# kai0511/insider

Measured on AMD Instinct MI355X. Metric: outer-iterations/sec (masked INSIDER fit, 10000 x 50000, K=30), higher is better.
Workload: dtype f64

## Files before the change

### insider_amd/csrc/insider_hip.hip

```cpp
#include "insider_kernels.hpp"
#include "insider_posthoc.hpp"
#include "insider_vardecomp.hpp"
#include "insider_sampdecomp.hpp"
#include "insider_levelscores.hpp"
#include "insider_factdecomp.hpp"
#include "insider_rescomp.hpp"
#include "insider_outliers.hpp"
#include "insider_neighbors.hpp"
#include "insider_coexpr.hpp"
#include "insider_enrich.hpp"
#include "insider_kmeans.hpp"
#include "insider_tsne.hpp"

#include <rccl/rccl.h>

#include <algorithm>
#include <chrono>
#include <cstdlib>
#include <cmath>
#include <cstdio>
#include <cstring>
#include <limits>
#include <memory>
#include <mutex>
// ... 222 lines not shown
    int blocks() const { return c + (m > 0 ? 1 : 0); }
    Block block(int b) const { return b < c ? Block{n_levels[b], lvl_off[b]} : Block{m, SLcat}; }

    DataSet() = default;
    DataSet(const DataSet &) = delete;
    DataSet &operator=(const DataSet &) = delete;
    ~DataSet() { (void)hipSetDevice(device); }
};

struct Workspace {
    static constexpr int EARLY = 3;
    int K = 0, NB = 0, KP = 0, nseg = 1;
    int gram_blocks_p = 0, gram_blocks_n = 0, sc_blocks = 0;
    DevBuf<double> Astack, R, C, RtR, CCt, Qfull, SC, stat, stat_col, gram_part, sc_part, lvl_part, eq, lvl_sum;
    DevBuf<double> fperm;
    DevBuf<double> lvl_zero;
    DevBuf<double> Qheld;
    DevBuf<double> U, Ylvl, wpart, Vlev;
    DevBuf<double> lvl_sum_all;
    DevBuf<double> gram_part2, sc_part2;
    DevBuf<double> wg_part;
    DevBuf<uint8_t> wg_pair;
    DevBuf<double> sse_train, sse_test, b2, b1, loss_buf, stage;
    size_t stage_count = 0;
    DevBuf<int> sweeps, failflag;
    DevBuf<int> sweep_key;
    DevBuf<unsigned long long> sweep_total;
    DevBuf<unsigned> pc4_ticket;
    unsigned pc4_base[2] = {0, 0};
    unsigned long long cd_code_base = 0, cd_pair_base = 0;
    DevBuf<unsigned long long> code_base_dev;
    uint8_t *order = nullptr;
    DevBuf<uint8_t> order_buf[2];
    int order_rows = 0;
    DevBuf<int> gene_perm;
    DevBuf<int> sched_cnt[2], sched_rank;
    DevBuf<uint16_t> sched_bkt;
    int sched_flip = 0;
    DevBuf<double> cd_hsave, cd_isave;
    DevBuf<uint32_t> cd_pass_slot;
    DevBuf<int> cd_pass_perm[2], cd_pass_cnt;
    DevBuf<int> perm_early[EARLY];
    bool have_early[EARLY] = {false, false, false};
    bool have_perm = false;
};

// ... 1 lines not shown

struct Join {
    Event ev;
    bool pending = false;
    int record(hipStream_t s) { HIPCHECK(hipEventRecord(ev, s)); pending = true; return INSIDER_OK; }
    int wait(hipStream_t s)
    {
        if (pending) HIPCHECK(hipStreamWaitEvent(s, ev, 0));
        pending = false;
        return INSIDER_OK;
    }
    void drop() { pending = false; }
};

struct Streams {
    Stream stream;
    Stream side;
    Stream side2;
    Stream side3;
    Event ev_cd_done, ev_prep, ev_c_ready;
    Event ev_head;
    std::vector<Event> ev_w;
    Event ev_a_ready, ev_tab;
    Join qfull, qheld, side_done;

    int create(int n_w)
    {
        HIPCHECK(hipStreamCreate(stream.out()));
        for (Stream *s : {&side, &side2, &side3}) HIPCHECK(hipStreamCreateWithFlags(s->out(), hipStreamNonBlocking));
        for (Event *e : {&ev_prep, &ev_c_ready, &ev_head, &ev_a_ready, &qfull.ev, &qheld.ev, &ev_cd_done, &side_done.ev, &ev_tab})
            HIPCHECK(hipEventCreateWithFlags(e->out(), EV_SYNC));
        ev_w.resize(n_w);
        for (Event &e : ev_w) HIPCHECK(hipEventCreateWithFlags(e.out(), EV_SYNC));
        return INSIDER_OK;
    }
    int synchronize_sides() const
    {
        for (const Stream *s : {&side, &side2, &side3}) HIPCHECK(hipStreamSynchronize(*s));
        return INSIDER_OK;
    }
    void synchronize() const
    {
        for (const Stream *s : {&stream, &side, &side2, &side3}) if (*s) (void)hipStreamSynchronize(*s);
    }
};

struct Options {
    int max_sweeps = 1 << 24, order_mode = 0, profile = 0, verbose = 0, cd_variant = 0, force_allreduce = 0;
    int col_factored = 1;
    int row_counts = 1;
    int row_merged = 1;
    int row_gemm = 1;
    int wg_waves = 1024;
    int row_fused = 1;
    int mm_fast = 1;
    int mm_tiles = 0;
    int col_mfma4 = 1;
    int cd_pairs = 1;
    int list_fine = 1;
    int cd_cold_iters = 3, cd_pass_first = 64, cd_pass_ratio = 4;
    double resid_stage_mb = 256.0;
    double vd_stage_kb = 48.0;
    int sd_slabs = 0;
    int ls_slabs = 0;
    double ls_part_mb = 256.0;
    int glm_slabs = 0;
    int rc_slabs = 0;
};

struct PostWs {
    DevBuf<double> Ast, U, cp, part, stats, stage, gpart, gram, cpart, gsum, L, dinv, outs;
    DevBuf<int> nz, ints, info;
    DevBuf<double> vin, vtab, vrec;
    DevBuf<double> spart, srec;
    DevBuf<double> lcand, ltab, lpart, lcnt, lout;
    DevBuf<double> fwall, fprod, fbase, frec;
    DevBuf<double> rq, rcs, rz, rpart, rin, rout;
    DevBuf<double> ocs, oz;
    DevBuf<uint32_t> obits;
    DevBuf<int> ogcnt, oscnt, orows, ocols;
    DevBuf<long long> ooffs;
};

}

struct insider_hip_handle {
    std::shared_ptr<const DataSet> ds;
    Streams st;
    Options opt;
    Workspace ws;
    PostWs post;
    FitPlan plan;
    bool w_ready = false;
    int64_t gene_offset = 0;
    int rank = 0, world = 1;
    insider_allreduce_fn allreduce = nullptr;
    void *allreduce_user = nullptr;
    ncclComm_t comm = nullptr;
    std::vector<Event> ev_col, ev_row, ev_cd, ev_test;
    double prof[12] = {0, 0, 0, 0, 0, 0, 0, 0, 0, 0, 0, 0};
    double steady_cd_ms = 0, steady_col_ms = 0;
    int cap_hits = 0, max_gene_sweeps = 0;
    int col_solver = 0, col_eval = 0, col_ridge_fallback = 0;
    int col_stats_kernel = 0, col_stats_tickets = 0, col_stats_blocks = 0;
    int col_q_kernel = 0, mm_rows2_tiles = 0;
    uint64_t row_kernels = 0;
    int vd_path = 0;
    int sd_path = 0, sd_slabs = 0;
    int ls_path = 0, ls_slabs = 0;
    int glm_slabs = 0, glm_form = 0;
    int fd_path = 0;
    int ls_form = 0, fd_form = 0, rc_form = 0, cx_form = 0;
    int rc_slabs = 0;
    double rc_ms = 0.0;
    double cx_stage_mb = 0.0, cx_stage_ms = 0.0, cx_ms = 0.0;
    int ol_path = 0;

    ~insider_hip_handle()
    {
        if (ds) (void)hipSetDevice(ds->device);
        st.synchronize();
        if (comm) (void)ncclCommDestroy(comm);
    }
};

namespace {

constexpr int PC4_PARTS = 16;
constexpr int MM_SLAB = 128;

enum RowKernel {
    RK_WGEMM4 = 0, RK_WGEMM5, RK_WGEMM6, RK_WGEMM7, RK_WGEMM_CHUNKS, RK_WSYRK, RK_GRAM_SIDE,
    RK_GENE_U_CNT, RK_GENE_U, RK_GENE_UC,
    RK_MERGED_SOLVE, RK_MERGED, RK_MERGED_ZERO, RK_PACK_REDUCE,
    RK_LIST_STATS4, RK_LIST_STATS, RK_LEVEL_PARTIAL, RK_LEVEL_SOLVE, RK_CONT_CD,
    RK_MM_ROWS2, RK_MM_ROWS, RK_MM_REDUCE2_2, RK_MM_REDUCE2_4, RK_MM_REDUCE
};
inline uint64_t rk_bit(RowKernel k) { return 1ull << (int)k; }
inline void row_mark(insider_hip_handle *h, RowKernel k) { h->row_kernels |= rk_bit(k); }

PlanFacts plan_facts(const insider_hip_handle *h, int K)
{
    const DataSet &d = *h->ds;
    PlanFacts f;
    const Options &o = h->opt;
    f.opt = {o.row_merged, o.col_factored, o.row_fused, o.row_gemm, o.row_counts, o.mm_fast, o.force_allreduce, o.wg_waves};
    f.world = h->world;
    f.K = K; f.NB = h->ws.NB; f.KP = h->ws.KP; f.lvl_zero = (bool)h->ws.lvl_zero;
    f.merged = d.merged; f.cont_merged = d.cont_merged; f.cf_pair_ok = d.cf_pair_ok; f.cf_hn = (bool)d.cf_hn; f.cf_zt = (bool)d.cf_zt;
    f.c = d.c; f.m = d.m; f.SL = d.SL; f.SLcat = d.SLcat; f.p = d.p; f.col_entries = d.col_entries; f.row_entries = d.row_entries;
    for (const CovTables &ct : d.cov) { f.L.push_back(ct.L); f.npairs.push_back(ct.npairs); }
    f.cf_c = d.cf.c; f.cf_tab_rows = d.cf.tab_rows; f.cf_nsteps = d.cf.nsteps;
// ... 58 lines not shown
            for (int a = 0; a < K; ++a)
                for (int b = 0; b <= a; ++b, ++idx) {
                    ab[idx] = (uint8_t)a;
                    ab[(size_t)16 * wg_ntile + idx] = (uint8_t)b;
                }
            if ((rc = w.wg_pair.upload(ab))) return rc;
        }
        if ((rc = w.U.alloc((size_t)d.p * round_up(max_L, 2)))) return rc;
        if ((rc = w.Ylvl.alloc(max_L * KP))) return rc;
        if ((rc = w.wpart.alloc((size_t)std::max(d.max_items, 1) * STAT))) return rc;
        if ((rc = w.lvl_sum_all.alloc((size_t)std::max(d.SL, 1) * rec))) return rc;
        if ((rc = w.gram_part2.alloc((size_t)std::max(w.gram_blocks_p, w.gram_blocks_n) * KP * KP))) return rc;
        if ((rc = w.sc_part2.alloc((size_t)w.sc_blocks * d.SL * KP))) return rc;
        if ((rc = w.Vlev.alloc((size_t)d.p * d.SLP))) return rc;
        HIPCHECK(hipMemsetAsync(w.Vlev, 0, (size_t)d.p * d.SLP * sizeof(double), st));
        if ((rc = w.Qheld.alloc((size_t)d.p * KP))) return rc;
    }
    if ((rc = w.eq.alloc((size_t)d.max_L * (KP * KP + KP)))) return rc;
    for (DevBuf<double> *b : {&w.sse_train, &w.sse_test, &w.b2, &w.b1})
        if ((rc = b->alloc((size_t)d.p))) return rc;
    if ((rc = w.loss_buf.alloc(8))) return rc;
    w.stage_count = (size_t)std::max<int64_t>(std::max<int64_t>(d.p, d.n), d.SL) * KP;
    if ((rc = w.stage.alloc(w.stage_count))) return rc;
    if ((rc = w.sweeps.alloc((size_t)d.p))) return rc;
    if ((rc = w.failflag.alloc(4))) return rc;
    if ((rc = w.sweep_total.alloc(256))) return rc;
    if ((rc = w.pc4_ticket.alloc((size_t)(PC4_PARTS + 1) * 32))) return rc;
    HIPCHECK(hipMemsetAsync(w.pc4_ticket, 0, (size_t)(PC4_PARTS + 1) * 32 * sizeof(unsigned), st));
    if ((rc = w.gene_perm.alloc((size_t)d.p))) return rc;
    if ((rc = w.sched_cnt[0].alloc((size_t)SCHED_BUCKETS))) return rc;
    if ((rc = w.sched_cnt[1].alloc((size_t)SCHED_BUCKETS))) return rc;
    if ((rc = w.sched_rank.alloc((size_t)d.p))) return rc;
    if ((rc = w.sched_bkt.alloc((size_t)d.p))) return rc;
    if ((rc = w.sweep_key.alloc((size_t)d.p))) return rc;
    if ((rc = w.cd_hsave.alloc((size_t)d.p * KP))) return rc;
    if ((rc = w.cd_isave.alloc((size_t)d.p * KP))) return rc;
    if ((rc = w.cd_pass_slot.alloc((size_t)d.p))) return rc;
    if ((rc = w.cd_pass_perm[0].alloc((size_t)d.p))) return rc;
    if ((rc = w.cd_pass_perm[1].alloc((size_t)d.p))) return rc;
    if ((rc = w.cd_pass_cnt.alloc((size_t)CD_BUCKETS + 2))) return rc;
    if ((rc = w.code_base_dev.alloc(2))) return rc;
    for (DevBuf<int> &b : w.perm_early)
        if ((rc = b.alloc((size_t)d.p))) return rc;
    HIPCHECK(hipMemsetAsync(w.sched_cnt[0], 0, SCHED_BUCKETS * sizeof(int), st));
    HIPCHECK(hipMemsetAsync(w.sched_cnt[1], 0, SCHED_BUCKETS * sizeof(int), st));
    HIPCHECK(hipMemsetAsync(w.C, 0, (size_t)(std::max<int64_t>(d.p, d.ldp) + 4) * KP * sizeof(double), st));
// ... 160 lines not shown

int phase_R(insider_hip_handle *h, bool use_side = false, bool r_is_current = false, bool want_qheld = false)
{
    if (use_side) {
        HIPCHECK(hipEventRecord(h->st.ev_a_ready, h->st.stream));
        HIPCHECK(hipStreamWaitEvent(h->st.side, h->st.ev_a_ready, 0));
        if (want_qheld && h->ws.Qheld && h->plan.col_path != 0) {
            HIPCHECK(hipStreamWaitEvent(h->st.side3, h->st.ev_a_ready, 0));
            if (int rh = launch_mm_rows_kp(h, h->ds->Sheld, h->ds->SLP, (int)h->ds->p, h->ds->SL, h->ws.Astack, h->ws.Qheld, h->st.side3)) return rh;
            if (int rh = h->st.qheld.record(h->st.side3)) return rh;
        }
        int rq = launch_mm_rows_kp(h, h->ds->S, h->ds->SLP, (int)h->ds->p, h->ds->SL, h->ws.Astack, h->ws.Qfull, h->st.side);
        if (rq) return rq;
        if ((rq = h->st.qfull.record(h->st.side))) return rq;
    }
    int rc = r_is_current ? INSIDER_OK : launch_build_R(h);
    if (rc) return rc;
    rc = launch_gram(h, h->ws.R, h->ds->n, h->ws.RtR);
    if (rc) return rc;
    if (use_side) return INSIDER_OK;
    return launch_mm_rows_kp(h, h->ds->S, h->ds->SLP, (int)h->ds->p, h->ds->SL, h->ws.Astack, h->ws.Qfull);
}

struct Timer {
    Event e0, e1;
    int begin(insider_hip_handle *h, bool on)
    {
        if (!on || !h->opt.profile) return INSIDER_OK;
        HIPCHECK(hipEventCreateWithFlags(e0.out(), hipEventDisableSystemFence));
        HIPCHECK(hipEventCreateWithFlags(e1.out(), hipEventDisableSystemFence));
        HIPCHECK(hipEventRecord(e0, h->st.stream));
        return INSIDER_OK;
    }
    int end(insider_hip_handle *h, std::vector<Event> &into)
    {
        if (!e0) return INSIDER_OK;
        HIPCHECK(hipEventRecord(e1, h->st.stream));
        into.push_back(std::move(e0));
        into.push_back(std::move(e1));
        return INSIDER_OK;
    }
};

struct Stopwatch {
    Event e0, e1;
    bool marked = false;
    int start(hipStream_t st)
    {
        if (!e0) {
            HIPCHECK(hipEventCreate(e0.out()));
            HIPCHECK(hipEventCreate(e1.out()));
        }
        marked = false;
        HIPCHECK(hipEventRecord(e0, st));
        return INSIDER_OK;
    }
    int mark(hipStream_t st)
    {
        HIPCHECK(hipEventRecord(e1, st));
        marked = true;
        return INSIDER_OK;
    }
// ... 191 lines not shown
        if (h->plan.col_path == 2) {
            a.cnt = h->ds->cf_cnt;
            a.hn = h->ds->cf_hn;
            a.zt = h->ds->cf_zt;
            rc = launch_paircnt(h, a);
            if (rc) return rc;
        } else {
            NB_DISPATCH(h->ws.NB, {
                (void)WPB_;
                const size_t lds = ((size_t)(a.tab_rows + 1) * Geo<NB_>::KP + (size_t)4 * 16 * 17) * sizeof(double) + (size_t)4 * CF_CAP * 2;
                hipLaunchKernelGGL((k_col_factored<NB_, 4>), dim3(cdiv(h->ds->p, 4)), dim3(256), lds, h->st.stream, a);
            });
            h->col_stats_kernel = CSK_FACTORED;
            h->col_stats_tickets = h->col_stats_blocks = 0;
        }
        KCHECK();
    } else {
        uint64_t mark = 0;
        rc = launch_list_stats(h, true, 1, h->ws.R, h->ws.stat_col, h->ws.RtR, &mark);
        if (rc) return rc;
        h->col_stats_kernel = (mark & rk_bit(RK_LIST_STATS4)) ? CSK_LIST4 : CSK_LIST;
        h->col_stats_tickets = h->col_stats_blocks = 0;
    }
    return t.end(h, h->ev_col);
}

template <typename Args>
void col_args_head(const insider_hip_handle *h, int masked, int checkpoint, Args &a)
{
    a.stat = masked ? h->ws.stat_col : nullptr;
    a.stat_len = h->plan.stat_len;
    a.p = (int)h->ds->p;
    a.K = h->ws.K;
    a.KP = h->ws.KP;
    a.RtR = h->ws.RtR;
    a.Qfull = h->ws.Qfull;
    a.C = h->ws.C;
    a.yy = masked ? h->ds->yy_train : h->ds->yy_all;
    a.checkpoint = checkpoint;
    a.sse_train = h->ws.sse_train;
    a.b2 = h->ws.b2;
    a.b1 = h->ws.b1;
    a.sse_test = h->ws.sse_test;
    a.test_from_stats = masked && h->ds->no_na;
}

int launch_col_solve(insider_hip_handle *h, int masked, bool solve, double lambda, double alpha, double tol,
                     int checkpoint, bool timed, int outer_iter = -1, bool side = false)
{
    const bool early = outer_iter >= 0 && outer_iter < Workspace::EARLY;
    int rc;
    if ((rc = h->st.side_done.wait(h->st.stream))) return rc;
    if ((rc = h->st.qfull.wait(h->st.stream))) return rc;
    Timer t;
    if ((rc = t.begin(h, timed))) return rc;
    bool eval_after = false, fused_bucket = false;
    ColArgs eval_args;
    h->col_solver = h->col_eval = h->col_ridge_fallback = CS_NONE;
    if (alpha == 0.0) {
        RidgeArgs a;
        col_args_head(h, masked, checkpoint, a);
        a.lambda = lambda;
        a.solve = solve ? 1 : 0;
        a.fail = h->ws.failflag;
        a.mark = h->ws.sweeps;
        a.retry = h->ws.failflag + 1;
        a.only_marked = 0;
        if (h->ws.K <= 32 && h->opt.cd_variant == 0) {
            if (solve) {
                HIPCHECK(hipMemsetAsync(h->ws.sweeps, 0, (size_t)h->ds->p * sizeof(int), h->st.stream));
                HIPCHECK(hipMemsetAsync(h->ws.failflag + 1, 0, sizeof(int), h->st.stream));
            }
            REG_DISPATCH(h->ws.K, hipLaunchKernelGGL((k_ridge_cols_reg<SL_, KM_>), dim3(cdiv(h->ds->p, 4)), dim3(64), 0, h->st.stream, a));
            h->col_solver = CS_RIDGE_REG;
            KCHECK();
            if (solve) {
                a.only_marked = 1;
                hipLaunchKernelGGL((k_ridge_cols<1>), dim3((unsigned)h->ds->p), dim3(64), 0, h->st.stream, a);
// ... 60 lines not shown
                if (solve) {
                    if ((rc = launch_cd(cs, a, h->st.stream))) return rc;
                    h->col_solver = cs;
                }
                if (!limit) break;
                int *count_out = h->ws.cd_pass_cnt + CD_BUCKETS + (pass & 1);
                hipLaunchKernelGGL(k_pass_scatter, dim3(cdiv(h->ds->p, 256)), dim3(256), 0, h->st.stream,
                                   (const uint32_t *)h->ws.cd_pass_slot, (const int *)h->ws.cd_pass_cnt, perm_in, a.pass_count, (int)h->ds->p,
                                   h->ws.cd_pass_perm[pass & 1], count_out);
                KCHECK();
                perm_in = a.gene_perm = h->ws.cd_pass_perm[pass & 1];
                a.pass_count = count_out;
                a.resume = 1;
                start = limit;
            }
            eval_after = checkpoint != 0;
            eval_args = a;
        } else {
            if ((rc = launch_cd(cs, a, h->st.stream))) return rc;
            h->col_solver = cs;
        }
    }
    if ((rc = t.end(h, h->ev_cd))) return rc;
    if (eval_after) {
        eval_args.gene_perm = nullptr;
        eval_args.pass_count = nullptr;
        eval_args.resume = 0;
        if (h->ws.K <= 32) {
            REG_DISPATCH(h->ws.K, hipLaunchKernelGGL((k_cd_cols_reg<SL_, KM_, false>), dim3(cdiv(h->ds->p, 4)), dim3(64), 0, h->st.stream, eval_args));
            h->col_eval = CS_CD_REG;
        } else {
            const size_t eb = (size_t)r16_lds_doubles(h->ws.K) * sizeof(double);
            if (int rl = r16_wide_lds(eb)) return rl;
            eval_args.mode = COL_EVAL;
            hipLaunchKernelGGL((k_cd_cols_r16<3>), dim3(cdiv(h->ds->p, 4)), dim3(64), eb, h->st.stream, eval_args);
            h->col_eval = CS_CD_R16_3;
        }
        KCHECK();
    }
    if (solve && alpha != 0.0) {
        hipStream_t st = h->st.stream;
        if (side) {
            HIPCHECK(hipEventRecord(h->st.ev_cd_done, h->st.stream));
            HIPCHECK(hipStreamWaitEvent(h->st.side, h->st.ev_cd_done, 0));
            st = h->st.side;
        }
// ... 296 lines not shown
        NB_DISPATCH(h->ws.NB, {
            (void)WPB_;
            hipLaunchKernelGGL((k_cont_cd<NB_>), dim3(1), dim3(64), 0, h->st.stream, (const double *)h->ws.eq, h->ws.K, lambda1,
                               h->ws.Astack + (size_t)row0 * h->ws.KP);
        });
        row_mark(h, RK_CONT_CD);
    } else {
        NB_DISPATCH(h->ws.NB, {
            (void)WPB_;
            hipLaunchKernelGGL((k_level_solve<NB_>), dim3(ct.L), dim3(64), 0, h->st.stream, (const double *)h->ws.eq,
                               (const int *)(cont ? h->ds->one_count : h->ds->lvl_count_all + h->ds->lvl_off[i]), ct.L, h->ws.K, lambda1,
                               h->ws.Astack + (size_t)row0 * h->ws.KP, h->ws.failflag);
        });
        row_mark(h, RK_LEVEL_SOLVE);
    }
    KCHECK();
    return rebuild_R ? launch_build_R(h) : INSIDER_OK;
}

struct LossOut {
    double sum_residual, train_rmse, test_rmse, row_reg_half, col_reg_half, l1_reg, loss;
};

int loss_checkpoint(insider_hip_handle *h, int tuning, double lambda1, double lambda2, double alpha, LossOut *o)
{
    hipLaunchKernelGGL(k_loss_reduce, dim3(1), dim3(256), 0, h->st.stream, h->ws.sse_train, h->ws.sse_test, h->ws.b2, h->ws.b1,
                       (int)h->ds->p, h->ws.Astack, h->ds->SL, h->ws.K, h->ws.KP, h->ws.loss_buf);
    KCHECK();
    double cnt[2] = {tuning == 1 ? h->ds->cnt_train : (double)h->ds->n * (double)h->ds->p, h->ds->cnt_test};
    HIPCHECK(hipMemcpyAsync(h->ws.loss_buf + 4, cnt, 2 * sizeof(double), hipMemcpyHostToDevice, h->st.stream));
    int rc = do_allreduce(h, h->ws.loss_buf, 6);
    if (rc) return rc;
    double v[8];
    HIPCHECK(hipMemcpyAsync(v, h->ws.loss_buf, 8 * sizeof(double), hipMemcpyDeviceToHost, h->st.stream));
    HIPCHECK(hipStreamSynchronize(h->st.stream));
    o->sum_residual = v[0];
    o->train_rmse = std::sqrt(v[0] / v[4]);
    o->test_rmse = (tuning == 1 && v[5] > 0) ? std::sqrt(v[1] / v[5]) : std::numeric_limits<double>::quiet_NaN();
    const double nfA = std::sqrt(v[6]), nfC = std::sqrt(v[2]);
    o->row_reg_half = lambda1 * nfA * nfA / 2;
    o->col_reg_half = lambda2 * (1 - alpha) * nfC * nfC / 2;
    o->l1_reg = lambda2 * alpha * v[3];
    o->loss = o->sum_residual / 2 + o->row_reg_half + o->col_reg_half + o->l1_reg;
    return INSIDER_OK;
}

int check_fail_flag(insider_hip_handle *h)
{
    int f = 0;
    HIPCHECK(hipMemcpyAsync(&f, h->ws.failflag, sizeof(int), hipMemcpyDeviceToHost, h->st.stream));
    HIPCHECK(hipStreamSynchronize(h->st.stream));
    if (f) {
        HIPCHECK(hipMemsetAsync(h->ws.failflag, 0, sizeof(int), h->st.stream));
        return fail(INSIDER_ERR_SOLVE, "a ridge normal-equation system was not positive definite");
    }
    return INSIDER_OK;
}

int read_cap_hits(insider_hip_handle *h)
{
    int v[2] = {0, 0};
    HIPCHECK(hipMemcpyAsync(v, h->ws.failflag + 2, sizeof(v), hipMemcpyDeviceToHost, h->st.stream));
    HIPCHECK(hipStreamSynchronize(h->st.stream));
    h->cap_hits = v[0];
    h->max_gene_sweeps = v[1];
    return INSIDER_OK;
}

void clear_events(insider_hip_handle *h)
{
    for (auto *v : {&h->ev_col, &h->ev_row, &h->ev_cd, &h->ev_test}) v->clear();
}

int upload_factors(insider_hip_handle *h, double *const *A, const double *C, int K)
{
    const DataSet &d = *h->ds;
    const int KP = h->ws.KP;
    const hipStream_t st = h->st.stream;
    for (int b = 0; b < d.blocks(); ++b) {
        const DataSet::Block blk = d.block(b);
        HIPCHECK(hipMemcpyAsync(h->ws.stage, A[b], (size_t)blk.rows * K * sizeof(double), hipMemcpyHostToDevice, st));
        hipLaunchKernelGGL(k_pack_A, dim3(cdiv(blk.rows * KP, 256)), dim3(256), 0, st, (const double *)h->ws.stage, blk.rows, K, KP,
                           h->ws.Astack + (size_t)blk.off * KP);
        KCHECK();
        HIPCHECK(hipStreamSynchronize(st));
    }
    if (!C) return INSIDER_OK;
    HIPCHECK(hipMemcpyAsync(h->ws.stage, C, (size_t)d.p * K * sizeof(double), hipMemcpyHostToDevice, st));
    hipLaunchKernelGGL(k_pack_rows, dim3(cdiv(d.p * KP, 256)), dim3(256), 0, st, (const double *)h->ws.stage, d.p, K, KP, h->ws.C);
    KCHECK();
    return INSIDER_OK;
}

int download_factors(insider_hip_handle *h, double *const *A, double *C, int K)
{
    const DataSet &d = *h->ds;
    const int KP = h->ws.KP;
    const hipStream_t st = h->st.stream;
    for (int b = 0; A && b < d.blocks(); ++b) {
        const DataSet::Block blk = d.block(b);
        hipLaunchKernelGGL(k_unpack_A, dim3(cdiv(blk.rows * K, 256)), dim3(256), 0, st,
                           (const double *)(h->ws.Astack + (size_t)blk.off * KP), blk.rows, K, KP, h->ws.stage);
        KCHECK();
        HIPCHECK(hipMemcpyAsync(A[b], h->ws.stage, (size_t)blk.rows * K * sizeof(double), hipMemcpyDeviceToHost, st));
        HIPCHECK(hipStreamSynchronize(st));
    }
    if (C) {
        hipLaunchKernelGGL(k_unpack_rows, dim3(cdiv(d.p * K, 256)), dim3(256), 0, st, (const double *)h->ws.C, d.p, K, KP,
                           h->ws.stage);
        KCHECK();
        HIPCHECK(hipMemcpyAsync(C, h->ws.stage, (size_t)d.p * K * sizeof(double), hipMemcpyDeviceToHost, st));
        HIPCHECK(hipStreamSynchronize(st));
    }
    return INSIDER_OK;
}

int launch_row_prep(insider_hip_handle *h)
{
    int rc = launch_gram(h, h->ws.C, h->ds->p, h->ws.CCt);
    if (rc) return rc;
    return launch_mm_reduce_kp(h, h->plan.merged ? h->ds->Strain : h->ds->S, h->ds->SLP, h->ws.C, (int)h->ds->p, h->ds->SL, h->ws.sc_part, h->ws.SC);
}

int check_factor_args(insider_hip_handle *h, double *const *A, const double *C, int inc_continuous, int tuning)
{
    if (!h || !A || !C) return fail(INSIDER_ERR_ARG, "null argument");
    if (tuning != 0 && tuning != 1)
        return fail(INSIDER_ERR_ARG, "Parameter tuning should be either 0 or 1!");
    if (inc_continuous != 0 && inc_continuous != 1)
        return fail(INSIDER_ERR_ARG, "The value of prarameter inc_continuous can only be 0 or 1.");
    if (inc_continuous == 1 && h->ds->m == 0)
        return fail(INSIDER_ERR_ARG, "inc_continuous = 1 needs a handle created with ctns_confounder (insider_hip_create_ex)");
    if (inc_continuous == 0 && h->ds->m > 0)
        return fail(INSIDER_ERR_ARG, "this handle carries continuous covariates: pass inc_continuous = 1");
    for (int b = 0; b < h->ds->blocks(); ++b) if (!A[b]) return fail(INSIDER_ERR_ARG, "null row factor");
    return INSIDER_OK;
// ... 723 lines not shown
{
    if (!h || !name) return fail(INSIDER_ERR_ARG, "null");
    const std::string s(name);
    if (s == "max_sweeps") h->opt.max_sweeps = value < 1 ? 1 : (int)value;
    else if (s == "order_mode") h->opt.order_mode = (int)value;
    else if (s == "profile") h->opt.profile = (int)value;
    else if (s == "verbose") h->opt.verbose = (int)value;
    else if (s == "force_allreduce") h->opt.force_allreduce = (int)value;
    else if (s == "col_factored") h->opt.col_factored = (int)value;
    else if (s == "row_counts") h->opt.row_counts = (int)value;
    else if (s == "row_merged") h->opt.row_merged = (int)value;
    else if (s == "row_gemm_waves") {
        h->opt.wg_waves = std::max(64, (int)value);
        HIPCHECK(hipSetDevice(h->ds->device));
        h->ws = Workspace();
    }
    else if (s == "row_gemm") h->opt.row_gemm = (int)value;
    else if (s == "row_fused") h->opt.row_fused = (int)value;
    else if (s == "cd_cold_iters") h->opt.cd_cold_iters = (int)value;
    else if (s == "cd_pass1") h->opt.cd_pass_first = (int)value;
    else if (s == "cd_pass_ratio") h->opt.cd_pass_ratio = (int)value;
    else if (s == "list_fine") h->opt.list_fine = (int)value;
    else if (s == "mm_fast") h->opt.mm_fast = (int)value;
    else if (s == "mm_tiles") h->opt.mm_tiles = value < 1 ? 0 : (int)value;
    else if (s == "col_mfma4") h->opt.col_mfma4 = (int)value;
    else if (s == "cd_pairs") h->opt.cd_pairs = (int)value;
    else if (s == "resid_stage_mb") h->opt.resid_stage_mb = value;
    else if (s == "vd_stage_kb") h->opt.vd_stage_kb = value;
    else if (s == "ls_slabs") h->opt.ls_slabs = value < 1 ? 0 : (int)std::min(value, 256.0);
    else if (s == "rc_slabs") h->opt.rc_slabs = value < 1 ? 0 : (int)std::min(value, 256.0);
    else if (s == "ls_part_mb") h->opt.ls_part_mb = value;
    else if (s == "glm_slabs") h->opt.glm_slabs = value < 1 ? 0 : (int)std::min(value, 64.0);
    else if (s == "sd_slabs") h->opt.sd_slabs = value < 1 ? 0 : (int)std::min(value, 256.0);
    else if (s == "cd_variant") h->opt.cd_variant = (int)value;
    else return fail(INSIDER_ERR_ARG, "unknown option " + s);
    return INSIDER_OK;
}

static void reset_call_state(insider_hip_handle *h, bool drain)
{
    if (drain) (void)hipSetDevice(h->ds->device);
    if (drain) h->st.synchronize();
    h->w_ready = false;
    for (Join *j : {&h->st.qfull, &h->st.qheld, &h->st.side_done}) j->drop();
    clear_events(h);
}

static double decay_for(double delta_loss)
{
    for (double d : {1e-6, 1e-5, 1e-4, 1e-3, 1e-2, 1e-1})
        if (delta_loss / 1000 <= d) return d;
    return 1.0;
}

static void profile_summary(insider_hip_handle *h, double wall_ms, double iterations, double sweeps_total)
{
    for (double &v : h->prof) v = 0;
    auto sum_events = [](std::vector<Event> &ev, size_t first, double *launches, double *ms) {
        for (size_t i = first; i + 1 < ev.size(); i += 2) {
            float t = 0;
            if (hipEventElapsedTime(&t, ev[i], ev[i + 1]) == hipSuccess) { *ms += t; *launches += 1; }
        }
    };
    sum_events(h->ev_col, 0, &h->prof[0], &h->prof[1]);
    sum_events(h->ev_row, 0, &h->prof[2], &h->prof[3]);
    sum_events(h->ev_cd, 0, &h->prof[4], &h->prof[5]);
    sum_events(h->ev_test, 0, &h->prof[6], &h->prof[7]);
    auto tail_mean = [&](std::vector<Event> &ev) {
        double ms = 0.0, cnt = 0.0;
        sum_events(ev, 10, &cnt, &ms);
        return cnt ? ms / cnt : 0.0;
    };
    h->steady_cd_ms = tail_mean(h->ev_cd);
    h->steady_col_ms = tail_mean(h->ev_col);
    h->prof[8] = wall_ms;
    h->prof[9] = iterations;
    h->prof[10] = sweeps_total;
    const FitPlan &p = h->plan;
    h->prof[11] = (p.masked && p.col_path != 0 ? 1.0 : 0.0) + (p.merged ? 2.0 : 0.0) + (p.masked && p.col_path == 2 ? 4.0 : 0.0);
    clear_events(h);
}

static int optimize_body(insider_hip_handle *h, double *const *A, double *C, int inc_continuous, int K, double lambda1,
                         double lambda2, double alpha, int tuning, double global_tol, double sub_tol, uint32_t max_iter,
                         uint64_t seed, double *out_train_rmse, double *out_test_rmse, double *out_loss, double *traj,
                         int traj_cap, int *out_traj_rows, int *out_iters)
{
    int rc = check_factor_args(h, A, C, inc_continuous, tuning);
    if (rc) return rc;
    HIPCHECK(hipSetDevice(h->ds->device));
    if ((rc = h->st.synchronize_sides())) return rc;
    if ((rc = ensure_workspace(h, K))) return rc;
    const auto t_begin = std::chrono::steady_clock::now();
    reset_call_state(h, false);
    h->row_kernels = 0;
    const int masked = tuning == 1;
    plan_call(h, masked);
    const FitPlan &plan = h->plan;
    if ((rc = upload_factors(h, A, C, K))) return rc;

    LossOut lo;
    if ((rc = phase_R(h))) return rc;
    if (masked) if ((rc = launch_col_stats(h, false))) return rc;
    if ((rc = launch_col_solve(h, masked, false, lambda2, alpha, sub_tol, 1, false))) return rc;
    if ((rc = launch_test_sse(h, masked, false))) return rc;
    if ((rc = loss_checkpoint(h, tuning, lambda1, lambda2, alpha, &lo))) return rc;
    double loss = lo.loss, pre_loss, decay = 1.0;
    double train_rmse = lo.train_rmse, test_rmse = lo.test_rmse;
    int trows = 0;
    auto put_traj = [&](double it, double delta, double dec) {
        if (traj && trows < traj_cap) {
            double *t = traj + (size_t)trows * INSIDER_TRAJ_STRIDE;
            t[0] = it; t[1] = lo.train_rmse; t[2] = lo.test_rmse; t[3] = lo.sum_residual / 2; t[4] = lo.row_reg_half;
            t[5] = lo.col_reg_half; t[6] = lo.l1_reg; t[7] = lo.loss; t[8] = delta; t[9] = dec;
            ++trows;
        }
    };
    put_traj(-1, std::numeric_limits<double>::quiet_NaN(), decay);

    uint32_t iter = 0;
    unsigned long long sweeps_total = 0;
    HIPCHECK(hipMemsetAsync(h->ws.sweep_total, 0, 256 * sizeof(unsigned long long), h->st.stream));
    HIPCHECK(hipMemsetAsync(h->ws.failflag + 2, 0, 2 * sizeof(int), h->st.stream));
    if (alpha != 0.0 && !h->ws.have_perm && !h->ws.have_early[0]) {
        hipLaunchKernelGGL(k_yy_key, dim3(cdiv(h->ds->p, 256)), dim3(256), 0, h->st.stream,
                           (const double *)(masked ? h->ds->yy_train : h->ds->yy_all), (int)h->ds->p, h->ws.sweep_key);
        KCHECK();
        if ((rc = launch_gene_order(h, nullptr, 0, 1, h->st.stream))) return rc;
        h->ws.have_perm = true;
    }
    while (iter <= max_iter) {
        if (h->opt.verbose && iter % 10 == 0) printf("Iteration %u ---------------------------------\n", iter);
        if (plan.merged) {
            if ((rc = launch_wsyrk_side(h))) return rc;
            if ((rc = launch_gene_v(h, h->ds->c > 1 ? h->ds->lvl_off[1] : h->ds->SLcat, h->ds->SL))) return rc;
            HIPCHECK(hipStreamWaitEvent(h->st.stream, h->st.ev_head, 0));
        } else {
            if ((rc = launch_row_prep(h))) return rc;
            if (masked) if ((rc = launch_row_stats(h, true))) return rc;
        }
        const bool cont_follow = inc_continuous && h->ds->m > 0;
        for (int i = 0; i < h->ds->c; ++i) {
            const bool need_R = !(plan.merged || plan.unmasked_fused) || (i + 1 == h->ds->c && !cont_follow);
            if ((rc = row_update(h, i, -1, masked, lambda1, need_R))) return rc;
// ... 1 lines not shown
                if ((rc = launch_gene_v(h, h->ds->lvl_off[i], h->ds->lvl_off[i + 1]))) return rc;
        }
        if (cont_follow)
            for (int j = 0; j < h->ds->m; ++j) {
                if ((rc = row_update(h, 0, j, masked, lambda1, !plan.merged || j + 1 == h->ds->m))) return rc;
                if (plan.merged && j + 1 < h->ds->m)
                    if ((rc = launch_gene_v(h, h->ds->SLcat + j, h->ds->SLcat + j + 1))) return rc;
            }
        h->w_ready = false;
        if ((rc = phase_R(h, true, true, masked != 0))) return rc;
        const int checkpoint = iter % 10 == 0;
        if (alpha != 0.0 && iter == 0)
            if ((rc = ensure_order_table(h, seed, iter, K, h->opt.max_sweeps, h->opt.order_mode, lambda2 * alpha, nullptr, 0))) return rc;
        if (masked) if ((rc = launch_col_stats(h, true))) return rc;
        if (alpha != 0.0) {
            h->ws.order = h->ws.order_buf[iter & 1];
            if (iter < max_iter) {
                HIPCHECK(hipEventRecord(h->st.ev_tab, h->st.stream));
                HIPCHECK(hipStreamWaitEvent(h->st.side, h->st.ev_tab, 0));
                if ((rc = ensure_order_table(h, seed, iter + 1, K, h->opt.max_sweeps, h->opt.order_mode, lambda2 * alpha, h->st.side, (int)((iter + 1) & 1))))
                    return rc;
            }
        }
        if ((rc = launch_col_solve(h, masked, true, lambda2, alpha, sub_tol * decay, checkpoint, true, (int)iter, true))) return rc;
        if (alpha != 0.0)
            if ((rc = side_close(h))) return rc;
        if (checkpoint) {
            if ((rc = launch_test_sse(h, masked, true))) return rc;
            pre_loss = loss;
            if ((rc = loss_checkpoint(h, tuning, lambda1, lambda2, alpha, &lo))) return rc;
            if ((rc = check_fail_flag(h))) return rc;
            loss = lo.loss;
            train_rmse = lo.train_rmse;
            test_rmse = lo.test_rmse;
            const double delta_loss = pre_loss - loss;
            decay = decay_for(delta_loss);
            put_traj(iter, delta_loss, decay);
            if (h->opt.verbose) {
                printf("insider iter %u: train rmse = %.12g\n", iter, train_rmse);
                if (tuning == 1) printf("insider iter %u: test rmse = %.12g\n", iter, test_rmse);
                printf("total_residual\t%.12g;\nrow_reg_loss:\t%.12g;\ncol_reg_loss:\t%.12g;\nl1_reg_loss:\t%.12g.\n",
                       lo.sum_residual / 2, lo.row_reg_half, lo.col_reg_half, lo.l1_reg);
                printf("Delta loss for iter %u:%.12g\n", iter, delta_loss);
            }
            if ((pre_loss - loss) / pre_loss < global_tol) break;
        }
        ++iter;
    }
    if ((rc = download_factors(h, A, C, K))) return rc;
    if ((rc = check_fail_flag(h))) return rc;
    if ((rc = read_cap_hits(h))) return rc;
    if ((rc = h->st.synchronize_sides())) return rc;
    h->st.side_done.drop();
    {
        unsigned long long bins[256];
        HIPCHECK(hipMemcpyAsync(bins, h->ws.sweep_total, sizeof(bins), hipMemcpyDeviceToHost, h->st.stream));
        HIPCHECK(hipStreamSynchronize(h->st.stream));
        for (unsigned long long v : bins) sweeps_total += v;
    }
    if (out_train_rmse) *out_train_rmse = train_rmse;
    if (out_test_rmse) *out_test_rmse = test_rmse;
    if (out_loss) *out_loss = loss;
    if (out_traj_rows) *out_traj_rows = trows;
    if (out_iters) *out_iters = (int)iter;
    profile_summary(h, std::chrono::duration<double, std::milli>(std::chrono::steady_clock::now() - t_begin).count(),
                    (double)std::min<uint64_t>((uint64_t)iter + 1, (uint64_t)max_iter + 1), (double)sweeps_total);
    return INSIDER_OK;
}

int insider_hip_optimize(insider_hip_handle *h, double *const *A, double *C, int inc_continuous, int K, double lambda1,
                         double lambda2, double alpha, int tuning, double global_tol, double sub_tol, uint32_t max_iter,
                         uint64_t seed, double *out_train_rmse, double *out_test_rmse, double *out_loss, double *traj,
                         int traj_cap, int *out_traj_rows, int *out_iters)
{
    const int rc = optimize_body(h, A, C, inc_continuous, K, lambda1, lambda2, alpha, tuning, global_tol, sub_tol, max_iter,
                                 seed, out_train_rmse, out_test_rmse, out_loss, traj, traj_cap, out_traj_rows, out_iters);
    if (rc != INSIDER_OK && h && h->st.stream) {
// ... 1949 lines not shown
```

### insider_amd/csrc/insider_kernels.hpp

```cpp
#pragma once

#include <hip/hip_runtime.h>
#include <stdint.h>

#include "../../include/insider_perm.h"

namespace insider {

typedef double d4 __attribute__((ext_vector_type(4)));
typedef double d2 __attribute__((ext_vector_type(2)));

constexpr int WAVE = 64;
constexpr int CHUNK = 128;

constexpr int LEVEL_CHUNK = 4;
#define INSIDER_ORDER_ROW 448
constexpr int ORDER_ROW = INSIDER_ORDER_ROW;

constexpr int CODE_TRAIN = 1;
constexpr int CODE_TEST = 2;

template <int NB>
struct Geo {
    static constexpr int KP = 16 * NB;
// ... 1442 lines not shown
    }
    S[(size_t)j * SLP + gl] = s;
}

__global__ void k_pack_rows(const double *__restrict__ src , int64_t len, int K, int KP,
                            double *__restrict__ dst)
{
    const int64_t t = (int64_t)blockIdx.x * blockDim.x + threadIdx.x;
    if (t >= len * KP) return;
    const int64_t r = t / KP;
    const int k = (int)(t % KP);
    dst[t] = k < K ? src[r * K + k] : 0.0;
}

__global__ void k_unpack_rows(const double *__restrict__ src, int64_t len, int K, int KP, double *__restrict__ dst)
{
    const int64_t t = (int64_t)blockIdx.x * blockDim.x + threadIdx.x;
    if (t >= len * K) return;
    const int64_t r = t / K;
    const int k = (int)(t % K);
    dst[t] = src[r * KP + k];
}

__global__ void k_pack_A(const double *__restrict__ src, int L, int K, int KP, double *__restrict__ dst_rows)
{
    const int t = blockIdx.x * blockDim.x + threadIdx.x;
    if (t >= L * KP) return;
    const int l = t / KP, k = t % KP;
    dst_rows[t] = k < K ? src[l + (size_t)k * L] : 0.0;
}

__global__ void k_unpack_A(const double *__restrict__ src_rows, int L, int K, int KP, double *__restrict__ dst)
{
    const int t = blockIdx.x * blockDim.x + threadIdx.x;
    if (t >= L * K) return;
    const int l = t % L, k = t / L;
    dst[t] = src_rows[(size_t)l * KP + k];
}

__device__ __forceinline__ double sumsq_or_zero(double v) { return v < 0.0 ? 0.0 : v; }

__global__ void __launch_bounds__(256) k_loss_reduce(const double *__restrict__ sse_train,
                                                     const double *__restrict__ sse_test, const double *__restrict__ b2,
                                                     const double *__restrict__ b1, int p,
                                                     const double *__restrict__ Astack, int SL, int K, int KP,
                                                     double *__restrict__ out)
// ... 103 lines not shown
```

Baseline: 689.7.

## Overlap C upload/download on side stream, merge end status reads, pool timer events

Moves the host-to-device upload and packing of C onto the side3 stream so it overlaps with the R phase and column stats. On the last checkpoint iteration, the unpack and download of C are enqueued on side3 before the loss read, so they overlap with it. The final fail-flag, cap-hit and sweep-bin reads are merged into one gather kernel plus a single copy, replacing several synchronous round trips. Profiling timers now reuse pooled events and share boundary events instead of creating new ones per call. This trades added event and stream dependencies, and some risk of ordering errors, for fewer serialized host syncs per fit call.

```diff
diff --git a/insider_amd/csrc/insider_hip.hip b/insider_amd/csrc/insider_hip.hip
--- a/insider_amd/csrc/insider_hip.hip
+++ b/insider_amd/csrc/insider_hip.hip
@@ -268,6 +268,8 @@
     DevBuf<double> wg_part;
     DevBuf<uint8_t> wg_pair;
     DevBuf<double> sse_train, sse_test, b2, b1, loss_buf, stage;
+    DevBuf<double> stage_c;
+    DevBuf<unsigned long long> status;
     size_t stage_count = 0;
     DevBuf<int> sweeps, failflag;
     DevBuf<int> sweep_key;
@@ -315,13 +317,17 @@
     Event ev_head;
     std::vector<Event> ev_w;
     Event ev_a_ready, ev_tab;
+    Event ev_xfer, ev_c_up;
+    Event ev_c_final;
+    Event ev_join[3];
     Join qfull, qheld, side_done;
 
     int create(int n_w)
     {
         HIPCHECK(hipStreamCreate(stream.out()));
         for (Stream *s : {&side, &side2, &side3}) HIPCHECK(hipStreamCreateWithFlags(s->out(), hipStreamNonBlocking));
-        for (Event *e : {&ev_prep, &ev_c_ready, &ev_head, &ev_a_ready, &qfull.ev, &qheld.ev, &ev_cd_done, &side_done.ev, &ev_tab})
+        for (Event *e : {&ev_prep, &ev_c_ready, &ev_head, &ev_a_ready, &qfull.ev, &qheld.ev, &ev_cd_done, &side_done.ev, &ev_tab, &ev_xfer, &ev_c_up,
+                         &ev_c_final, &ev_join[0], &ev_join[1], &ev_join[2]})
             HIPCHECK(hipEventCreateWithFlags(e->out(), EV_SYNC));
         ev_w.resize(n_w);
         for (Event &e : ev_w) HIPCHECK(hipEventCreateWithFlags(e.out(), EV_SYNC));
@@ -359,6 +365,9 @@
     double ls_part_mb = 256.0;
     int glm_slabs = 0;
     int rc_slabs = 0;
+    int xfer_overlap = 1;
+    int status_merged = 1;
+    int timer_pool = 1;
 };
 
 struct PostWs {
@@ -390,7 +399,11 @@
     insider_allreduce_fn allreduce = nullptr;
     void *allreduce_user = nullptr;
     ncclComm_t comm = nullptr;
-    std::vector<Event> ev_col, ev_row, ev_cd, ev_test;
+    std::vector<hipEvent_t> ev_col, ev_row, ev_cd, ev_test;
+    std::vector<Event> ev_pool;
+    size_t ev_next = 0;
+    hipEvent_t ev_shared = nullptr;
+    bool mark_c_final = false;
     double prof[12] = {0, 0, 0, 0, 0, 0, 0, 0, 0, 0, 0, 0};
     double steady_cd_ms = 0, steady_col_ms = 0;
     int cap_hits = 0, max_gene_sweeps = 0;
@@ -421,6 +434,7 @@
 
 constexpr int PC4_PARTS = 16;
 constexpr int MM_SLAB = 128;
+constexpr int STATUS_HEAD = 4;
 
 enum RowKernel {
     RK_WGEMM4 = 0, RK_WGEMM5, RK_WGEMM6, RK_WGEMM7, RK_WGEMM_CHUNKS, RK_WSYRK, RK_GRAM_SIDE,
@@ -525,6 +539,8 @@
     if ((rc = w.loss_buf.alloc(8))) return rc;
     w.stage_count = (size_t)std::max<int64_t>(std::max<int64_t>(d.p, d.n), d.SL) * KP;
     if ((rc = w.stage.alloc(w.stage_count))) return rc;
+    if ((rc = w.stage_c.alloc((size_t)d.p * KP))) return rc;
+    if ((rc = w.status.alloc(STATUS_HEAD + 256))) return rc;
     if ((rc = w.sweeps.alloc((size_t)d.p))) return rc;
     if ((rc = w.failflag.alloc(4))) return rc;
     if ((rc = w.sweep_total.alloc(256))) return rc;
@@ -731,22 +747,38 @@
     return launch_mm_rows_kp(h, h->ds->S, h->ds->SLP, (int)h->ds->p, h->ds->SL, h->ws.Astack, h->ws.Qfull);
 }
 
+int timer_event(insider_hip_handle *h, hipEvent_t *out)
+{
+    if (h->ev_next == h->ev_pool.size()) {
+        h->ev_pool.emplace_back();
+        HIPCHECK(hipEventCreateWithFlags(h->ev_pool.back().out(), hipEventDisableSystemFence));
+    }
+    *out = h->ev_pool[h->ev_next++];
+    return INSIDER_OK;
+}
+
 struct Timer {
-    Event e0, e1;
-    int begin(insider_hip_handle *h, bool on)
+    hipEvent_t e0 = nullptr, e1 = nullptr;
+    int begin(insider_hip_handle *h, bool on, bool adjoins = false)
     {
+        const hipEvent_t prev = h->ev_shared;
+        h->ev_shared = nullptr;
         if (!on || !h->opt.profile) return INSIDER_OK;
-        HIPCHECK(hipEventCreateWithFlags(e0.out(), hipEventDisableSystemFence));
-        HIPCHECK(hipEventCreateWithFlags(e1.out(), hipEventDisableSystemFence));
-        HIPCHECK(hipEventRecord(e0, h->st.stream));
-        return INSIDER_OK;
-    }
-    int end(insider_hip_handle *h, std::vector<Event> &into)
+        if (adjoins && prev && h->opt.timer_pool) {
+            e0 = prev;
+        } else {
+            if (int rc = timer_event(h, &e0)) return rc;
+            HIPCHECK(hipEventRecord(e0, h->st.stream));
+        }
+        return timer_event(h, &e1);
+    }
+    int end(insider_hip_handle *h, std::vector<hipEvent_t> &into, bool share = false)
     {
         if (!e0) return INSIDER_OK;
         HIPCHECK(hipEventRecord(e1, h->st.stream));
-        into.push_back(std::move(e0));
-        into.push_back(std::move(e1));
+        into.push_back(e0);
+        into.push_back(e1);
+        if (share) h->ev_shared = e1;
         return INSIDER_OK;
     }
 };
@@ -984,7 +1016,7 @@
         h->col_stats_kernel = (mark & rk_bit(RK_LIST_STATS4)) ? CSK_LIST4 : CSK_LIST;
         h->col_stats_tickets = h->col_stats_blocks = 0;
     }
-    return t.end(h, h->ev_col);
+    return t.end(h, h->ev_col, true);
 }
 
 template <typename Args>
@@ -1015,7 +1047,7 @@
     if ((rc = h->st.side_done.wait(h->st.stream))) return rc;
     if ((rc = h->st.qfull.wait(h->st.stream))) return rc;
     Timer t;
-    if ((rc = t.begin(h, timed))) return rc;
+    if ((rc = t.begin(h, timed, true))) return rc;
     bool eval_after = false, fused_bucket = false;
     ColArgs eval_args;
     h->col_solver = h->col_eval = h->col_ridge_fallback = CS_NONE;
@@ -1122,6 +1154,7 @@
         }
     }
     if ((rc = t.end(h, h->ev_cd))) return rc;
+    if (h->mark_c_final) HIPCHECK(hipEventRecord(h->st.ev_c_final, h->st.stream));
     if (eval_after) {
         eval_args.gene_perm = nullptr;
         eval_args.pass_count = nullptr;
@@ -1464,15 +1497,18 @@
     double sum_residual, train_rmse, test_rmse, row_reg_half, col_reg_half, l1_reg, loss;
 };
 
-int loss_checkpoint(insider_hip_handle *h, int tuning, double lambda1, double lambda2, double alpha, LossOut *o)
+int loss_enqueue(insider_hip_handle *h, int tuning)
 {
     hipLaunchKernelGGL(k_loss_reduce, dim3(1), dim3(256), 0, h->st.stream, h->ws.sse_train, h->ws.sse_test, h->ws.b2, h->ws.b1,
                        (int)h->ds->p, h->ws.Astack, h->ds->SL, h->ws.K, h->ws.KP, h->ws.loss_buf);
     KCHECK();
     double cnt[2] = {tuning == 1 ? h->ds->cnt_train : (double)h->ds->n * (double)h->ds->p, h->ds->cnt_test};
     HIPCHECK(hipMemcpyAsync(h->ws.loss_buf + 4, cnt, 2 * sizeof(double), hipMemcpyHostToDevice, h->st.stream));
-    int rc = do_allreduce(h, h->ws.loss_buf, 6);
-    if (rc) return rc;
+    return do_allreduce(h, h->ws.loss_buf, 6);
+}
+
+int loss_read(insider_hip_handle *h, int tuning, double lambda1, double lambda2, double alpha, LossOut *o)
+{
     double v[8];
     HIPCHECK(hipMemcpyAsync(v, h->ws.loss_buf, 8 * sizeof(double), hipMemcpyDeviceToHost, h->st.stream));
     HIPCHECK(hipStreamSynchronize(h->st.stream));
@@ -1487,6 +1523,12 @@
     return INSIDER_OK;
 }
 
+int loss_checkpoint(insider_hip_handle *h, int tuning, double lambda1, double lambda2, double alpha, LossOut *o)
+{
+    if (int rc = loss_enqueue(h, tuning)) return rc;
+    return loss_read(h, tuning, lambda1, lambda2, alpha, o);
+}
+
 int check_fail_flag(insider_hip_handle *h)
 {
     int f = 0;
@@ -1512,6 +1554,9 @@
 void clear_events(insider_hip_handle *h)
 {
     for (auto *v : {&h->ev_col, &h->ev_row, &h->ev_cd, &h->ev_test}) v->clear();
+    h->ev_next = 0;
+    h->ev_shared = nullptr;
+    if (!h->opt.timer_pool) h->ev_pool.clear();
 }
 
 int upload_factors(insider_hip_handle *h, double *const *A, const double *C, int K)
@@ -1554,6 +1599,62 @@
         HIPCHECK(hipMemcpyAsync(C, h->ws.stage, (size_t)d.p * K * sizeof(double), hipMemcpyDeviceToHost, st));
         HIPCHECK(hipStreamSynchronize(st));
     }
+    return INSIDER_OK;
+}
+
+int upload_C_side(insider_hip_handle *h, const double *C, int K)
+{
+    const DataSet &d = *h->ds;
+    const hipStream_t s3 = h->st.side3;
+    HIPCHECK(hipStreamWaitEvent(s3, h->st.ev_xfer, 0));
+    HIPCHECK(hipMemcpyAsync(h->ws.stage_c, C, (size_t)d.p * K * sizeof(double), hipMemcpyHostToDevice, s3));
+    hipLaunchKernelGGL(k_pack_rows, dim3(cdiv(d.p * h->ws.KP, 256)), dim3(256), 0, s3, (const double *)h->ws.stage_c, d.p, K, h->ws.KP,
+                       h->ws.C);
+    KCHECK();
+    HIPCHECK(hipEventRecord(h->st.ev_c_up, s3));
+    HIPCHECK(hipStreamWaitEvent(h->st.stream, h->st.ev_c_up, 0));
+    return INSIDER_OK;
+}
+
+int download_C_side(insider_hip_handle *h, double *C, int K)
+{
+    const DataSet &d = *h->ds;
+    const hipStream_t s3 = h->st.side3;
+    HIPCHECK(hipStreamWaitEvent(s3, h->st.ev_c_final, 0));
+    hipLaunchKernelGGL(k_unpack_rows, dim3(cdiv(d.p * K, 256)), dim3(256), 0, s3, (const double *)h->ws.C, d.p, K, h->ws.KP,
+                       h->ws.stage_c);
+    KCHECK();
+    HIPCHECK(hipMemcpyAsync(C, h->ws.stage_c, (size_t)d.p * K * sizeof(double), hipMemcpyDeviceToHost, s3));
+    return INSIDER_OK;
+}
+
+int join_sides(insider_hip_handle *h)
+{
+    const Stream *sides[3] = {&h->st.side, &h->st.side2, &h->st.side3};
+    for (int i = 0; i < 3; ++i) {
+        HIPCHECK(hipEventRecord(h->st.ev_join[i], *sides[i]));
+        HIPCHECK(hipStreamWaitEvent(h->st.stream, h->st.ev_join[i], 0));
+    }
+    return INSIDER_OK;
+}
+
+int read_status(insider_hip_handle *h, unsigned long long *sweeps_total)
+{
+    int rc = join_sides(h);
+    if (rc) return rc;
+    unsigned long long rec[STATUS_HEAD + 256];
+    hipLaunchKernelGGL(k_gather_status, dim3(1), dim3(256), 0, h->st.stream, (const int *)h->ws.failflag, STATUS_HEAD,
+                       (const unsigned long long *)h->ws.sweep_total, 256, (unsigned long long *)h->ws.status);
+    KCHECK();
+    HIPCHECK(hipMemcpyAsync(rec, h->ws.status, sizeof(rec), hipMemcpyDeviceToHost, h->st.stream));
+    HIPCHECK(hipStreamSynchronize(h->st.stream));
+    if (rec[0]) {
+        HIPCHECK(hipMemsetAsync(h->ws.failflag, 0, sizeof(int), h->st.stream));
+        return fail(INSIDER_ERR_SOLVE, "a ridge normal-equation system was not positive definite");
+    }
+    h->cap_hits = (int)(unsigned)rec[2];
+    h->max_gene_sweeps = (int)(unsigned)rec[3];
+    for (int b = 0; b < 256; ++b) *sweeps_total += rec[STATUS_HEAD + b];
     return INSIDER_OK;
 }
 
@@ -2323,6 +2424,9 @@
     else if (s == "cd_pass_ratio") h->opt.cd_pass_ratio = (int)value;
     else if (s == "list_fine") h->opt.list_fine = (int)value;
     else if (s == "mm_fast") h->opt.mm_fast = (int)value;
+    else if (s == "xfer_overlap") h->opt.xfer_overlap = (int)value;
+    else if (s == "status_merged") h->opt.status_merged = (int)value;
+    else if (s == "timer_pool") h->opt.timer_pool = (int)value;
     else if (s == "mm_tiles") h->opt.mm_tiles = value < 1 ? 0 : (int)value;
     else if (s == "col_mfma4") h->opt.col_mfma4 = (int)value;
     else if (s == "cd_pairs") h->opt.cd_pairs = (int)value;
@@ -2344,6 +2448,7 @@
     if (drain) h->st.synchronize();
     h->w_ready = false;
     for (Join *j : {&h->st.qfull, &h->st.qheld, &h->st.side_done}) j->drop();
+    h->mark_c_final = false;
     clear_events(h);
 }
 
@@ -2357,7 +2462,7 @@
 static void profile_summary(insider_hip_handle *h, double wall_ms, double iterations, double sweeps_total)
 {
     for (double &v : h->prof) v = 0;
-    auto sum_events = [](std::vector<Event> &ev, size_t first, double *launches, double *ms) {
+    auto sum_events = [](std::vector<hipEvent_t> &ev, size_t first, double *launches, double *ms) {
         for (size_t i = first; i + 1 < ev.size(); i += 2) {
             float t = 0;
             if (hipEventElapsedTime(&t, ev[i], ev[i + 1]) == hipSuccess) { *ms += t; *launches += 1; }
@@ -2367,7 +2472,7 @@
     sum_events(h->ev_row, 0, &h->prof[2], &h->prof[3]);
     sum_events(h->ev_cd, 0, &h->prof[4], &h->prof[5]);
     sum_events(h->ev_test, 0, &h->prof[6], &h->prof[7]);
-    auto tail_mean = [&](std::vector<Event> &ev) {
+    auto tail_mean = [&](std::vector<hipEvent_t> &ev) {
         double ms = 0.0, cnt = 0.0;
         sum_events(ev, 10, &cnt, &ms);
         return cnt ? ms / cnt : 0.0;
@@ -2398,11 +2503,14 @@
     const int masked = tuning == 1;
     plan_call(h, masked);
     const FitPlan &plan = h->plan;
-    if ((rc = upload_factors(h, A, C, K))) return rc;
+    const bool overlap = h->opt.xfer_overlap != 0;
+    HIPCHECK(hipEventRecord(h->st.ev_xfer, h->st.stream));
+    if ((rc = upload_factors(h, A, overlap ? nullptr : C, K))) return rc;
 
     LossOut lo;
     if ((rc = phase_R(h))) return rc;
     if (masked) if ((rc = launch_col_stats(h, false))) return rc;
+    if (overlap) if ((rc = upload_C_side(h, C, K))) return rc;
     if ((rc = launch_col_solve(h, masked, false, lambda2, alpha, sub_tol, 1, false))) return rc;
     if ((rc = launch_test_sse(h, masked, false))) return rc;
     if ((rc = loss_checkpoint(h, tuning, lambda1, lambda2, alpha, &lo))) return rc;
@@ -2421,6 +2529,7 @@
 
     uint32_t iter = 0;
     unsigned long long sweeps_total = 0;
+    bool c_down = false;
     HIPCHECK(hipMemsetAsync(h->ws.sweep_total, 0, 256 * sizeof(unsigned long long), h->st.stream));
     HIPCHECK(hipMemsetAsync(h->ws.failflag + 2, 0, 2 * sizeof(int), h->st.stream));
     if (alpha != 0.0 && !h->ws.have_perm && !h->ws.have_early[0]) {
@@ -2468,14 +2577,23 @@
                     return rc;
             }
         }
-        if ((rc = launch_col_solve(h, masked, true, lambda2, alpha, sub_tol * decay, checkpoint, true, (int)iter, true))) return rc;
+        const bool last = iter == max_iter;
+        h->mark_c_final = overlap && last && checkpoint;
+        rc = launch_col_solve(h, masked, true, lambda2, alpha, sub_tol * decay, checkpoint, true, (int)iter, true);
+        h->mark_c_final = false;
+        if (rc) return rc;
         if (alpha != 0.0)
             if ((rc = side_close(h))) return rc;
         if (checkpoint) {
             if ((rc = launch_test_sse(h, masked, true))) return rc;
             pre_loss = loss;
-            if ((rc = loss_checkpoint(h, tuning, lambda1, lambda2, alpha, &lo))) return rc;
-            if ((rc = check_fail_flag(h))) return rc;
+            if ((rc = loss_enqueue(h, tuning))) return rc;
+            if (overlap && last) {
+                if ((rc = download_C_side(h, C, K))) return rc;
+                c_down = true;
+            }
+            if ((rc = loss_read(h, tuning, lambda1, lambda2, alpha, &lo))) return rc;
+            if (!(last && h->opt.status_merged)) if ((rc = check_fail_flag(h))) return rc;
             loss = lo.loss;
             train_rmse = lo.train_rmse;
             test_rmse = lo.test_rmse;
@@ -2493,12 +2611,15 @@
         }
         ++iter;
     }
-    if ((rc = download_factors(h, A, C, K))) return rc;
-    if ((rc = check_fail_flag(h))) return rc;
-    if ((rc = read_cap_hits(h))) return rc;
-    if ((rc = h->st.synchronize_sides())) return rc;
-    h->st.side_done.drop();
-    {
+    if ((rc = download_factors(h, A, c_down ? nullptr : C, K))) return rc;
+    if (h->opt.status_merged) {
+        if ((rc = read_status(h, &sweeps_total))) return rc;
+        h->st.side_done.drop();
+    } else {
+        if ((rc = check_fail_flag(h))) return rc;
+        if ((rc = read_cap_hits(h))) return rc;
+        if ((rc = h->st.synchronize_sides())) return rc;
+        h->st.side_done.drop();
         unsigned long long bins[256];
         HIPCHECK(hipMemcpyAsync(bins, h->ws.sweep_total, sizeof(bins), hipMemcpyDeviceToHost, h->st.stream));
         HIPCHECK(hipStreamSynchronize(h->st.stream));
diff --git a/insider_amd/csrc/insider_kernels.hpp b/insider_amd/csrc/insider_kernels.hpp
--- a/insider_amd/csrc/insider_kernels.hpp
+++ b/insider_amd/csrc/insider_kernels.hpp
@@ -1488,6 +1488,14 @@
     dst[t] = src[r * KP + k];
 }
 
+__global__ void __launch_bounds__(256) k_gather_status(const int *__restrict__ flags, int nflag,
+                                                       const unsigned long long *__restrict__ bins, int nbins,
+                                                       unsigned long long *__restrict__ rec)
+{
+    for (int t = threadIdx.x; t < nflag + nbins; t += blockDim.x)
+        rec[t] = t < nflag ? (unsigned long long)(unsigned)flags[t] : bins[t - nflag];
+}
+
 __global__ void k_pack_A(const double *__restrict__ src, int L, int K, int KP, double *__restrict__ dst_rows)
 {
     const int t = blockIdx.x * blockDim.x + threadIdx.x;
```

Result: no change. 687.3 (-0.4%).
